# raviraina/grok

Measured on AMD Instinct MI355X. Metric: Mpixels/s encode+decode, 8K RGB 5/3 lossless + 9/7 lossy, 1/2/4/8 GPU, higher is better.
Workload: dtype int32 (5/3) + f32 (9/7)

## Files before the change

grok_amd/csrc/gk_engine.cpp:

```cpp
#include <hip/hip_runtime.h>

#include <algorithm>
#include <array>
#include <tuple>
#include <cmath>
#include <cstdarg>
#include <cstdlib>
#include <cstdio>
#include <cstring>
#include <memory>
#include <string>
#include <atomic>
#include <chrono>
#include <condition_variable>
#include <functional>
#include <mutex>
#include <thread>
#include <unordered_map>
#include <vector>
#include <queue>
#include <map>
#include <climits>
#include <linux/futex.h>
#include <sys/syscall.h>
// ... 2833 lines not shown
            } else if (p > q) {
                const uint32_t new_max = h.sgnd ? 1u << (p - 1) : (1u << p) - 1;
                const uint32_t old_max = h.sgnd ? 1u << (q - 1) : (1u << q) - 1;
                h.op = GK_PIX_SCALE;
                h.scale = (float)new_max / (float)old_max;
            } else if (p < q) {
                h.op = GK_PIX_SHIFT;
                h.shift = q - p;
            }
        }
    }
    return D;
}

}

struct DevBuf {
    void* p = nullptr; size_t cap = 0;
    void* get(size_t n) {
        if (n > cap) {
            if (p) (void)hipFree(p);
            p = nullptr; cap = 0;
            size_t c = std::max(n, (size_t)1 << 20);
            HIPCHK(hipMalloc(&p, c));
            cap = c;
        }
        return p;
    }
    ~DevBuf() { if (p) (void)hipFree(p); }
};
struct HostBuf {
    void* p = nullptr; size_t cap = 0;
    void* get(size_t n) {
        if (n > cap) {
            if (p) (void)hipHostFree(p);
            p = nullptr; cap = 0;
            size_t c = std::max(n, (size_t)1 << 20);
            HIPCHK(hipHostMalloc(&p, c, 0));
            cap = c;
        }
        return p;
    }
    ~HostBuf() { if (p) (void)hipHostFree(p); }
};

struct gk_ctx {
    uint32_t dec_layers = 0;
    bool dec_colour = true, col_inner = false, col_whole = false;
    uint32_t dec_display = 0;
    bool disp_inner = false;
    std::vector<gk_precision> dec_prec;
    bool out_inner = false;
    struct PixDst { void* pixels; size_t row_bytes; };
    const PixDst* pix = nullptr;
    DisplayOut hdr_disp;
    Jp2Colour hdr_col;
    ColourOut hdr_out;
    uint32_t hdr_ncs = 0;
    std::vector<uint8_t> col_blob;
    bool dwt_partial = false;
    uint32_t dec_reduce = 0;
    bool win_whole_tile = false;
    int device = 0;
    bool registered = false;
    hipStream_t st = nullptr;
    hipStream_t aux[3] = {nullptr, nullptr, nullptr};
    hipEvent_t xev[6];
    std::string err;
    gk_timings tm{};
    std::string plan_key;
    Plan plan;
    DevBuf arena;
    DevBuf bytes;
    DevBuf dblocks;
    DevBuf dpasses;
    DevBuf dinfo;
    DevBuf dseg;
    DevBuf dout;
    DevBuf dplanes;
    DevBuf derr;
    DevBuf dsym, dsymoff, dpassend, dcminfo;
    DevBuf dmsstate, dseglen;
    DevBuf dscratch, dnmse, dord, dweight, dord_enc;
    HostBuf hinfo, hseg, hhdr, hpasses, hord, hweight, hord_enc;
    DevBuf dstage1, dstage2;
    DevBuf dcol_src, dcol_out, dcol_tab;
    DevBuf dpix_src, dpix_out;
    DevBuf dicc_tab;
    std::vector<uint8_t> icc_blob;
    DevBuf dpix_in;
    HostBuf hstage1, hstage2;
    int16_t* nmse_tab = nullptr;
    hipEvent_t ev[32];
    bool blocks_uploaded = false;
    uint32_t enc_b0 = 0, enc_b1 = 0;
    std::vector<uint8_t> enc_dx, enc_dy;
    EncColour enc_col;
    std::vector<uint8_t> enc_jp2h;
    std::vector<uint32_t> hdr_dx, hdr_dy, hdr_prec, hdr_sgnd;
    bool enc_rc = false;
    std::vector<std::pair<uint32_t, uint32_t>> native_qcd, band_qcd;
    std::vector<gk_band_result> rb_bands;
    std::vector<gk_block_result> rb_blocks;
    std::vector<gk_pass_result> rb_passes;
    std::vector<uint8_t> rb_data;
};

static void set_params(Params& P, const gk_cparameters* cp, uint32_t nc) {
    for (int i = 0; i < GK_MAXRLVLS; ++i) { P.prcw[i] = 15; P.prch[i] = 15; }
    if (!cp) return;
    if (cp->numresolution > GK_MAXRLVLS) throw GkError("numresolution must be at most 33");
    if (cp->res_spec > GK_MAXRLVLS) throw GkError("res_spec must be at most 33");
    P.numres = cp->numresolution ? cp->numresolution : 6;
    P.cbw = (uint32_t)floorlog2(cp->cblockw_init ? cp->cblockw_init : 64);
    P.cbh = (uint32_t)floorlog2(cp->cblockh_init ? cp->cblockh_init : 64);
    P.irrev = cp->irreversible ? 1 : 0;
    P.mct = cp->mct;
    P.numgbits = cp->numgbits ? cp->numgbits : 2;
    P.nlayers = cp->numlayers ? cp->numlayers : 1;
    if (P.nlayers > GK_MAX_LAYERS) P.nlayers = GK_MAX_LAYERS;
    P.quality = cp->allocationByQuality != 0;
    for (uint32_t l = 0; l < GK_MAX_LAYERS; ++l) {
        P.rates[l] = (l < P.nlayers && !P.quality && cp->layer_rate[l] > 0.0) ? cp->layer_rate[l] : 0.0;
        P.dist[l] = (l < P.nlayers && P.quality && cp->layer_distortion[l] > 0.0) ? cp->layer_distortion[l] : 0.0;
    }
    if (cp->csty & ~7u) throw GkError("unknown coding style bits (csty)");
    P.sop_eph = cp->csty & 6u;
    P.write_com = cp->write_comment;
    P.comments.clear();
    if (cp->num_comments > GK_NUM_COMMENTS) throw GkError("at most 256 comments");
    uint32_t kept = 0;
    for (uint32_t i = 0; i < cp->num_comments; ++i)
        if (cp->comment_len[i] && cp->comment[i]) ++kept;
    for (uint32_t i = 0; i < kept; ++i) {
        if (!cp->comment_len[i] || !cp->comment[i]) continue;
        if (cp->comment_len[i] > 65531) throw GkError("comment longer than a COM marker holds (65531 bytes)");
        P.comments.push_back({cp->is_binary_comment[i] ? 0u : 1u, std::string(cp->comment[i], cp->comment_len[i])});
    }
    P.cblk_sty = cp->cblk_sty;
    if (cp->prog_order < 0 || cp->prog_order > 4) throw GkError("unknown progression order");
    P.prog = (uint32_t)cp->prog_order;
    P.roishift.clear();
    if (cp->roi_compno >= 0 && (uint32_t)cp->roi_compno < nc && cp->roi_shift) {
        if (cp->roi_shift >= 32) throw GkError("ROI shift must be below 32");
        P.roishift.assign(nc, 0);
        P.roishift[(size_t)cp->roi_compno] = (uint8_t)cp->roi_shift;
    }
    if (cp->numpocs > 32) throw GkError("at most 32 progression order changes");
    P.pocs.clear();
    for (uint32_t i = 0; i < cp->numpocs; ++i) {
        const gk_poc& g = cp->pocs[i];
        if (g.prog < 0 || g.prog > 4 || g.resE > GK_MAXRLVLS || g.resS >= g.resE || g.compS >= g.compE || !g.layE ||
            g.layE > 65535 || g.compE > 16384)
            throw GkError("bad progression order change");
        Poc e; e.rs = g.resS; e.cs = g.compS; e.lye = g.layE; e.re = g.resE; e.ce = g.compE; e.prog = (uint32_t)g.prog;
        P.pocs.push_back(e);
    }
    P.tp_div = cp->enableTilePartGeneration ? cp->newTilePartProgressionDivider : 0;
    if (P.tp_div && P.tp_div != 'L' && P.tp_div != 'R' && P.tp_div != 'C')
        throw GkError("tile-part divider must be L, R or C");
    if (cp->tile_size_on) {
        if (!cp->t_width || !cp->t_height) throw GkError("tile size must be non-zero when tiling is on");
        P.tw = cp->t_width; P.th = cp->t_height;
    }
    P.tlm = cp->writeTLM != 0; P.plt = cp->writePLT != 0;
    if (cp->cod_format != 0 && cp->cod_format != 2) throw GkError("cod_format must be GRK_CODEC_J2K (0) or GRK_CODEC_JP2 (2)");
    P.jp2 = cp->cod_format == 2;
// ... 342 lines not shown
        for (uint32_t c = 0; c < P.nc; ++c) {
            const Region& R = RGg[P.group_of[c]];
            const uint8_t* first = (const uint8_t*)comps[c] + (size_t)R.y0 * strides[c] * es;
            if (comps_on_device) { src[c] = first; sstr[c] = strides[c]; continue; }
            HIPCHK(hipMemcpy2DAsync(dp + o * es, (size_t)R.w * es, first, (size_t)strides[c] * es, (size_t)R.w * es, R.h,
                                    hipMemcpyHostToDevice, st));
            src[c] = dp + o * es; sstr[c] = R.w;
            o += (size_t)R.w * R.h;
        }
    }
    launch_check(__LINE__);
    HIPCHK(hipEventRecord(ctx->ev[1], st));
    int32_t shift = P.sgnd ? 0 : (1 << (P.prec - 1));
    auto planeA = [&](uint32_t c) { return arena + (size_t)c * 2 * RG.plane; };
    auto planeAf = [&](uint32_t c) { return reinterpret_cast<float*>(planeA(c)); };
    const bool mct3 = P.mct3();
    if (mct3 && (sstr[1] != sstr[0] || sstr[2] != sstr[0])) throw GkError("the first three components must share a stride");
    L1Io io;
    const bool fused = P.p.numres > 1 && P.l1_fusable;
    if (fused) {
        io.stype = stype; io.mct3 = mct3; io.shift.assign(P.nc, shift);
        io.planes.assign(src.begin(), src.end());
        io.strides = sstr;
    } else {
        auto cw = [&](uint32_t c) { return RGg[P.group_of[c]].w; };
        auto ch = [&](uint32_t c) { return RGg[P.group_of[c]].h; };
        if (!P.p.irrev) {
            if (mct3) gk_launch_dc_rct_fwd(st, stype, src[0], src[1], src[2], sstr[0], planeA(0), planeA(1), planeA(2), RG.stride, cw(0), ch(0), shift);
            for (uint32_t c = mct3 ? 3 : 0; c < P.nc; ++c) gk_launch_dc_fwd(st, stype, src[c], sstr[c], planeA(c), RG.stride, cw(c), ch(c), shift);
        } else {
            if (mct3) gk_launch_dc_ict_fwd(st, stype, src[0], src[1], src[2], sstr[0], planeAf(0), planeAf(1), planeAf(2), RG.stride, cw(0), ch(0), shift);
            for (uint32_t c = mct3 ? 3 : 0; c < P.nc; ++c) gk_launch_dc_fwd_f(st, stype, src[c], sstr[c], planeAf(c), RG.stride, cw(c), ch(c), shift);
        }
    }
    launch_check(__LINE__);
    HIPCHK(hipEventRecord(ctx->ev[2], st));
    run_dwt(ctx, RG, true, jb, je, 0, 0xffffffffu, fused ? &io : nullptr);
    if (const char* dp = getenv("GK_DUMP_DWT")) {
        std::vector<int32_t> hv((size_t)P.nc * 2 * RG.plane);
        HIPCHK(hipMemcpyAsync(hv.data(), arena, hv.size() * 4, hipMemcpyDeviceToHost, st));
        HIPCHK(hipStreamSynchronize(st));
        if (FILE* f = fopen(dp, "wb")) {
            const uint32_t hd[4] = {P.nc, RG.stride, RG.h, RG.w};
            fwrite(hd, 4, 4, f);
            fwrite(hv.data(), 4, hv.size(), f);
            fclose(f);
        }
    }
    launch_check(__LINE__);
    HIPCHK(hipEventRecord(ctx->ev[3], st));
    const bool do_rc = P.p.rate_control();
    const uint64_t slot0 = P.blocks[b0].data_off;
    const uint64_t slot1 = b1 < nb ? P.blocks[b1].data_off : P.slot_bytes;
    const uint64_t slot_span = slot1 - slot0;
    uint8_t* dbytes = (uint8_t*)ctx->bytes.get(slot_span + (64u << 20));
    const uint32_t nbx = std::max(nbr, 1u);
    GkBlock* dblk = (GkBlock*)ctx->dblocks.get(sizeof(GkBlock) * nbx);
    GkPass* dps = (GkPass*)ctx->dpasses.get(sizeof(GkPass) * GK_MAX_PASSES * (size_t)nbx);
    uint32_t* dinfo = (uint32_t*)ctx->dinfo.get(16 * (size_t)nbx + 16);
    int* derr = (int*)ctx->derr.get(64);
    uint32_t* dpcount = (uint32_t*)(derr + 4);
    uint8_t* dsym = P.p.ht() ? nullptr : (uint8_t*)ctx->dsym.get(P.sym_off[b1] - P.sym_off[b0] + 256);
    uint64_t* dsymoff = (uint64_t*)ctx->dsymoff.get(8 * ((size_t)nbr + 1));
    uint32_t* dpe = (uint32_t*)ctx->dpassend.get(4 * GK_MAX_PASSES * (size_t)nbx);
    uint32_t* dcm = (uint32_t*)ctx->dcminfo.get(8 * (size_t)nbx);
    int32_t* dnmse = do_rc ? (int32_t*)ctx->dnmse.get(4 * GK_MAX_PASSES * (size_t)nbx) : nullptr;
    if (!ctx->blocks_uploaded || ctx->enc_b0 != b0 || ctx->enc_b1 != b1 || ctx->enc_rc != do_rc) {
        GkBlock* hb = (GkBlock*)ctx->hpasses.get(sizeof(GkBlock) * nbx + 8 * ((size_t)nbr + 1));
        uint64_t* hso = (uint64_t*)(hb + nbx);
        for (uint32_t i = 0; i < nbr; ++i) {
            hb[i] = P.blocks[b0 + i];
            hb[i].band_off = relocate(P, group_region(P, RG, P.groups[P.group_of[hb[i].comp]]), hb[i].band_off);
            hb[i].stride = RG.stride;
            hb[i].data_off -= slot0;
            hb[i].flags = (uint8_t)((hb[i].flags & ~2u) | (do_rc ? 2u : 0u));
        }
        for (uint32_t i = 0; i <= nbr; ++i) hso[i] = P.sym_off[b0 + i] - P.sym_off[b0];
        HIPCHK(hipMemcpyAsync(dblk, hb, sizeof(GkBlock) * nbr, hipMemcpyHostToDevice, st));
        HIPCHK(hipMemcpyAsync(dsymoff, hso, 8 * ((size_t)nbr + 1), hipMemcpyHostToDevice, st));
        HIPCHK(hipStreamSynchronize(st));
        ctx->blocks_uploaded = true; ctx->enc_b0 = b0; ctx->enc_b1 = b1; ctx->enc_rc = do_rc;
    }
    HIPCHK(hipMemsetAsync(derr, 0, 64, st));
    const uint32_t nsolo_env = []() { const char* v = getenv("GK_T1ENC_SOLO"); return v ? (uint32_t)atoi(v) : 0u; }();
    if (P.p.ht()) {
        uint8_t* mel = (uint8_t*)ctx->dsym.get((size_t)nbx * GK_HT_MEL_CAP + 256);
        launch_check(__LINE__);
        HIPCHK(hipEventRecord(ctx->ev[8], st));
        gk_launch_ht_enc(st, arena, dblk, dbytes, mel, GK_HT_MEL_CAP, dinfo, nbr, derr, P.p.wide());
    } else if (P.p.t1_generic()) {
        uint8_t* mst = (uint8_t*)ctx->dmsstate.get(gk_t1ms_state_bytes(nbx));
        launch_check(__LINE__);
        HIPCHK(hipEventRecord(ctx->ev[8], st));
        gk_launch_t1_enc_ms(st, arena, dblk, dbytes, dps, dinfo, nbr, derr, ctx->nmse_tab, dpcount, mst, P.p.cblk_sty & 0x3f);
    } else if (nbr < 8192 || getenv("GK_T1ENC_SERIAL")) {
        gk_launch_t1_cm(st, arena, dblk, dsymoff, dsym, dpe, dcm, nbr, derr, ctx->nmse_tab, dnmse);
        launch_check(__LINE__);
        HIPCHK(hipEventRecord(ctx->ev[8], st));
        gk_launch_t1_mq(st, dsym, dsymoff, dpe, dcm, dblk, dbytes, dps, dinfo, nbr, derr, dnmse, dpcount, nullptr, 0,
                        0xffffffffu, std::min(nsolo_env, nbr));
    } else {
        uint32_t* dw = (uint32_t*)ctx->dweight.get(4 * (size_t)nbr);
        gk_launch_t1_weight(st, arena, dblk, dw, nbr);
        uint32_t* hw = (uint32_t*)ctx->hweight.get(4 * (size_t)nbr);
        HIPCHK(hipMemcpyAsync(hw, dw, 4 * (size_t)nbr, hipMemcpyDeviceToHost, st));
        HIPCHK(hipStreamSynchronize(st));
        uint32_t wmax = 1;
        for (uint32_t i = 0; i < nbr; ++i) wmax = std::max(wmax, hw[i]);
        const uint32_t kB = 4096;
        auto key = [&](uint32_t i) { return kB - 1 - (uint32_t)(((uint64_t)hw[i] * (kB - 1)) / wmax); };
        std::vector<uint32_t> start(kB + 1, 0);
        for (uint32_t i = 0; i < nbr; ++i) start[key(i)]++;
        for (uint32_t k = 0, acc = 0; k <= kB; ++k) { const uint32_t c = start[k]; start[k] = acc; acc += c; }
        uint32_t* ho = (uint32_t*)ctx->hord_enc.get(4 * (size_t)nbr);
        for (uint32_t i = 0; i < nbr; ++i) ho[start[key(i)]++] = i;
        uint32_t* dord = (uint32_t*)ctx->dord_enc.get(4 * (size_t)nbr);
        HIPCHK(hipMemcpyAsync(dord, ho, 4 * (size_t)nbr, hipMemcpyHostToDevice, st));
        static std::vector<double> frs[2];
        std::vector<double>& fr = frs[do_rc ? 1 : 0];
        if (fr.empty()) {
            const char* cv = getenv("GK_T1ENC_CUTS");
            std::string cs = cv ? cv : (do_rc ? "0.08,0.25" : "0.125,0.375");
            for (size_t q = 0; q < cs.size();) {
                size_t e = cs.find(',', q);
                if (e == std::string::npos) e = cs.size();
                const double f = atof(cs.substr(q, e - q).c_str());
                if (f > 0 && f < 1 && fr.size() < 3) fr.push_back(f);
                q = e + 1;
            }
        }
        std::vector<uint32_t> cut(1, 0);
        for (double f : fr) {
            const uint32_t c = (uint32_t)(nbr * f) / 256 * 256;
            if (c > cut.back() && c < nbr) cut.push_back(c);
        }
        cut.push_back(nbr);
        const int nch = (int)cut.size() - 1;
        for (int k = 0; k < nch; ++k) {
            const uint32_t base = cut[k], cnt = cut[k + 1] - cut[k];
            gk_launch_t1_cm(st, arena, dblk, dsymoff, dsym, dpe, dcm, nbr, derr, ctx->nmse_tab, dnmse, dord, base, cnt);
            if (k + 1 < nch) {
                HIPCHK(hipEventRecord(ctx->xev[k], st));
                HIPCHK(hipStreamWaitEvent(ctx->aux[k], ctx->xev[k], 0));
                gk_launch_t1_mq(ctx->aux[k], dsym, dsymoff, dpe, dcm, dblk, dbytes, dps, dinfo, nbr, derr, dnmse, dpcount,
                                dord, base, cnt, k == 0 ? std::min(nsolo_env, cnt) : 0u);
                HIPCHK(hipEventRecord(ctx->xev[3 + k], ctx->aux[k]));
            } else {
                launch_check(__LINE__);
                HIPCHK(hipEventRecord(ctx->ev[8], st));
                gk_launch_t1_mq(st, dsym, dsymoff, dpe, dcm, dblk, dbytes, dps, dinfo, nbr, derr, dnmse, dpcount, dord,
                                base, cnt);
            }
        }
        for (int k = 0; k + 1 < nch; ++k) HIPCHK(hipStreamWaitEvent(st, ctx->xev[3 + k], 0));
    }
    launch_check(__LINE__);
    HIPCHK(hipEventRecord(ctx->ev[4], st));
    static const bool eprof = getenv("GK_PROFILE") != nullptr;
    using eclk = std::chrono::steady_clock;
    auto ems = [](eclk::time_point a, eclk::time_point b) { return std::chrono::duration<double, std::milli>(b - a).count(); };
    const auto te0 = eclk::now();
    uint32_t* hinfo = (uint32_t*)ctx->hinfo.get(16 * (size_t)nb + 64);
    HIPCHK(hipMemcpyAsync(hinfo + 4 * (size_t)b0, dinfo, 16 * (size_t)nbr, hipMemcpyDeviceToHost, st));
    HIPCHK(hipMemcpyAsync(hinfo + 4 * (size_t)nb, derr, 32, hipMemcpyDeviceToHost, st));
    HIPCHK(hipStreamSynchronize(st));
    const uint32_t t1err = hinfo[4 * (size_t)nb], npass_total = hinfo[4 * (size_t)nb + 4];
    if (t1err) throw GkError(t1err & 2 ? "T1 symbol buffer overflow" : "T1 code-block slot overflow");
    const bool ht = P.p.ht();
    const GkPass* hpasses = nullptr;
    if ((do_rc || (P.p.cblk_sty & (GK_STY_LAZY | GK_STY_TERMALL))) && !ht) {
        GkPass* hp = (GkPass*)ctx->hpasses.get(sizeof(GkPass) * (size_t)std::max(npass_total, 1u));
        HIPCHK(hipMemcpyAsync(hp, dps, sizeof(GkPass) * (size_t)npass_total, hipMemcpyDeviceToHost, st));
        HIPCHK(hipStreamSynchronize(st));
        hpasses = hp;
    }
    if (blocks_only) {
        dump_blocks(ctx, hinfo, dps, npass_total, dbytes, slot0);
        *rc = 0;
        return 0;
    }

    std::vector<uint8_t> H;
    H.reserve(1 << 12);
    size_t tlm_pos = 0;
    write_main_header(H, P, &tlm_pos);
    const size_t rc_header_size = H.size() + (P.p.jp2 ? jp2_prefix_size(P, ctx->enc_jp2h) : 0);
    if (!with_header) H.clear();
    const auto te1 = eclk::now();
    if (const char* ds = getenv("GK_DUMP_SYMS"); ds && dsym && !P.p.t1_generic()) {
        std::vector<uint32_t> pe((size_t)GK_MAX_PASSES * nbr), cm(2 * (size_t)nbr), out(2 * (size_t)nbr);
        HIPCHK(hipMemcpy(pe.data(), dpe, 4 * pe.size(), hipMemcpyDeviceToHost));
        HIPCHK(hipMemcpy(cm.data(), dcm, 4 * cm.size(), hipMemcpyDeviceToHost));
        for (uint32_t i = 0; i < nbr; ++i) {
            out[2 * i] = cm[2 * i + 1] ? pe[(size_t)GK_MAX_PASSES * i + cm[2 * i + 1] - 1] : 0;
            out[2 * i + 1] = cm[2 * i];
        }
        if (FILE* f = fopen(ds, "wb")) { fwrite(out.data(), 4, out.size(), f); fclose(f); }
    }
    if (const char* dp = getenv("GK_DUMP_PASSES")) {
        if (FILE* f = fopen(dp, "wb")) {
            const uint32_t hdr[2] = {nb, npass_total};
            fwrite(hdr, 4, 2, f);
            fwrite(hinfo, 16, nb, f);
            if (hpasses) fwrite(hpasses, sizeof(GkPass), npass_total, f);
            fclose(f);
        }
    }
    T2Enc T2(P, hinfo, hpasses, tb, te);
    std::vector<T2Enc::Swallow> tsw(te - tb);
    if (te - tb == 1 || !P.p.rate_control()) {
        T2.allocate(rc_header_size);
        tsw[0] = T2.final_sw;
    } else {
        const bool par = te - tb >= host_pool().size();
        auto one = [&](size_t q) {
            const uint32_t t = tb + (uint32_t)q;
            T2Enc Tt(P, hinfo, hpasses, t, t + 1);
            Tt.serial = par;
            Tt.allocate(rc_header_size);
            tsw[q] = Tt.final_sw;
            const TileG& TG = P.tiles[t];
            std::copy(Tt.lnp.begin() + (size_t)TG.b0 * T2.L, Tt.lnp.begin() + (size_t)TG.b1 * T2.L,
                      T2.lnp.begin() + (size_t)TG.b0 * T2.L);
        };
        if (par) host_pool().run(te - tb, one);
        else for (uint32_t q = 0; q < te - tb; ++q) one(q);
    }
    const auto te2 = eclk::now();
// ... 2777 lines not shown
```

grok_amd/csrc/gk_launch.h:

```cpp
#pragma once
#include <hip/hip_runtime.h>
#include <stdint.h>
#include "gk_common.h"

#define GK_SAMPLE_DISPATCH(t, T, ...)                            \
    switch (t) {                                                 \
        case GK_U8: { typedef uint8_t T; __VA_ARGS__; break; }   \
        case GK_S8: { typedef int8_t T; __VA_ARGS__; break; }    \
        case GK_U16: { typedef uint16_t T; __VA_ARGS__; break; } \
        case GK_S16: { typedef int16_t T; __VA_ARGS__; break; }  \
        default: { typedef int32_t T; __VA_ARGS__; break; }      \
    }

void gk_launch_dc_rct_fwd(hipStream_t st, int stype, const void* r, const void* g, const void* b, uint32_t sin,
                          int32_t* y, int32_t* u, int32_t* v, uint32_t sout, uint32_t w, uint32_t h, int32_t shift);
void gk_launch_dc_fwd(hipStream_t st, int stype, const void* in, uint32_t sin, int32_t* out, uint32_t sout, uint32_t w,
                      uint32_t h, int32_t shift);
void gk_launch_rct_inv_dc(hipStream_t st, const int32_t* y, const int32_t* u, const int32_t* v, uint32_t sin, int stype,
                          void* r, void* g, void* b, uint32_t sout, uint32_t w, uint32_t h, int32_t shift,
                          int32_t mn, int32_t mx);
void gk_launch_dc_inv(hipStream_t st, const int32_t* in, uint32_t sin, int stype, void* out, uint32_t sout, uint32_t w,
                      uint32_t h, int32_t shift, int32_t mn, int32_t mx);
uint32_t gk_dwt_cpw(uint32_t wgs, uint32_t n, bool multi);
void gk_launch_dwt53_fwd(hipStream_t st, const int32_t* src, uint32_t sstride, int32_t* dst, uint32_t dstride,
                         uint32_t w, uint32_t h, GkTiles tb = GkTiles(), GkComps cs = GkComps());
void gk_launch_dwt53_inv(hipStream_t st, const int32_t* src, uint32_t sstride, int32_t* dst, uint32_t dstride,
                         uint32_t w, uint32_t h, GkTiles tb = GkTiles(), GkComps cs = GkComps());
void gk_launch_dwt53_fwd_l1(hipStream_t st, int stype, int nc, GkPtr3 in, uint32_t sin, int32_t* dst, uint64_t cstride,
                            uint32_t dstride, uint32_t w, uint32_t h, GkTiles tb, int32_t shift);
void gk_launch_dwt53_inv_l1(hipStream_t st, int stype, int nc, const int32_t* src, uint64_t cstride, uint32_t sstride,
                            GkPtr3 out, uint32_t ostride, GkWin win, uint32_t w, uint32_t h, GkTiles tb, int32_t shift,
                            int32_t mn, int32_t mx);
void gk_launch_gather(hipStream_t st, const uint8_t* src, uint8_t* dst, const uint64_t* seg, uint32_t nseg);
void gk_launch_t1_cm(hipStream_t st, const int32_t* coef, const GkBlock* blocks, const uint64_t* sym_off, uint8_t* sym,
                     uint32_t* pass_end, uint32_t* cm_info, uint32_t nblocks, int* err, const int16_t* nmse_tab,
                     int32_t* pass_nmse, const uint32_t* order = nullptr, uint32_t base = 0, uint32_t count = 0xffffffffu);
void gk_launch_t1_mq(hipStream_t st, const uint8_t* sym, const uint64_t* sym_off, const uint32_t* pass_end,
                     const uint32_t* cm_info, const GkBlock* blocks, uint8_t* bytes, GkPass* passes, uint32_t* info,
                     uint32_t nblocks, int* err, const int32_t* pass_nmse, uint32_t* pass_counter,
                     const uint32_t* order = nullptr, uint32_t base = 0, uint32_t count = 0xffffffffu,
                     uint32_t nsolo = 0);
void gk_launch_t1_weight(hipStream_t st, const int32_t* coef, const GkBlock* blocks, uint32_t* weight, uint32_t nblocks);
uint32_t gk_t1dec_lanes();
void gk_t1dec_stats(uint64_t out[5]);
struct GkSoloPlan { uint32_t waves; int forced; float ratio; };
GkSoloPlan gk_t1dec_solo_plan(uint32_t nblocks, uint32_t lanes);
void gk_launch_t1_dec(hipStream_t st, const uint8_t* bytes, const GkBlock* blocks, const uint32_t* order,
                      uint64_t* scratch, const uint64_t* wave_off, uint32_t nblocks, uint32_t nsolo);
void gk_launch_t1_recon(hipStream_t st, const GkBlock* blocks, const uint32_t* ids, const uint32_t* pos,
                        const uint64_t* scratch, const uint64_t* wave_off, int32_t* coef, uint32_t nblocks,
                        uint32_t maxnp);
void gk_launch_dwt_any(hipStream_t st, bool irrev, bool forward, int32_t* in, int32_t* out, uint32_t stride, uint32_t w,
                       uint32_t h, uint32_t px, uint32_t py, GkTiles tb, GkComps cs, bool partial = false);
void gk_launch_t1_enc_ms(hipStream_t st, const int32_t* coef, const GkBlock* blocks, uint8_t* bytes, GkPass* passes,
                         uint32_t* info, uint32_t nblocks, int* err, const int16_t* nmse_tab, uint32_t* pass_counter,
                         uint8_t* state, uint32_t sty);
void gk_launch_t1_dec_ms(hipStream_t st, const uint8_t* bytes, const GkBlock* blocks, const uint32_t* seglen, int32_t* coef,
                         uint32_t nblocks, uint8_t* state, uint32_t sty);
size_t gk_t1ms_state_bytes(uint32_t nblocks);
void gk_launch_dc_ict_fwd(hipStream_t st, int stype, const void* r, const void* g, const void* b, uint32_t sin, float* y,
                          float* u, float* v, uint32_t sout, uint32_t w, uint32_t h, int32_t shift);
void gk_launch_dc_fwd_f(hipStream_t st, int stype, const void* in, uint32_t sin, float* out, uint32_t sout, uint32_t w,
                        uint32_t h, int32_t shift);
void gk_launch_ict_inv_dc(hipStream_t st, const float* y, const float* u, const float* v, uint32_t sin, int stype, void* r,
                          void* g, void* b, uint32_t sout, uint32_t w, uint32_t h, int32_t shift, int32_t mn,
                          int32_t mx);
void gk_launch_dc_inv_f(hipStream_t st, const float* in, uint32_t sin, int stype, void* out, uint32_t sout, uint32_t w,
                        uint32_t h, int32_t shift, int32_t mn, int32_t mx);
void gk_launch_dwt97_fwd(hipStream_t st, const float* src, uint32_t sstride, float* dst, uint32_t dstride, uint32_t w,
                         uint32_t h, GkTiles tb = GkTiles(), GkComps cs = GkComps());
void gk_launch_dwt97_inv(hipStream_t st, const float* src, uint32_t sstride, float* dst, uint32_t dstride, uint32_t w,
                         uint32_t h, GkTiles tb = GkTiles(), GkComps cs = GkComps());
void gk_launch_dwt97_fwd_l1(hipStream_t st, int stype, int nc, GkPtr3 in, uint32_t sin, float* dst, uint64_t cstride,
                            uint32_t dstride, uint32_t w, uint32_t h, GkTiles tb, int32_t shift);
void gk_launch_dwt97_inv_l1(hipStream_t st, int stype, int nc, const float* src, uint64_t cstride, uint32_t sstride,
                            GkPtr3 out, uint32_t ostride, GkWin win, uint32_t w, uint32_t h, GkTiles tb, int32_t shift,
                            int32_t mn, int32_t mx);
void gk_launch_ht_enc(hipStream_t st, const int32_t* coef, const GkBlock* blocks, uint8_t* bytes, uint8_t* mel_scratch,
                      uint32_t mel_cap, uint32_t* info, uint32_t nblocks, int* err, bool wide = false);
void gk_launch_ht_dec(hipStream_t st, const uint8_t* bytes, const GkBlock* blocks, const uint32_t* ids, int32_t* coef,
                      uint32_t nblocks, int* err, bool wide = false);
struct GkPalChan {
    void* dst;
    const void* src;
    uint32_t dst_stride, src_stride;
    uint32_t col, direct;
};
struct GkPalArgs {
    const void* idx;
    uint32_t idx_stride;
    uint32_t w, h;
    const GkPalChan* chans;
    uint32_t nchan, npal;
    const uint32_t* table;
    uint32_t ne, entry_words, elem_bytes;
    uint32_t vec_store;
    uint32_t rows;
};
#define GK_PAL_PIX 8
#define GK_PAL_LDS_BYTES 65536u
uint32_t gk_pal_entry_words(uint32_t npc, uint32_t elem_bytes);
int gk_launch_jp2_palette(hipStream_t st, int stype, int dtype, const GkPalArgs& args);
enum GkYccMode { GK_YCC_444 = 0, GK_YCC_422 = 1, GK_YCC_420 = 2, GK_YCC_ESYCC = 3 };
struct GkYccArgs {
    const void* y; const void* cb; const void* cr;
    uint32_t ys, cs;
    void* dst[3];
    uint32_t ds[3];
    uint32_t w, h;
    uint32_t mode;
    uint32_t ofx, ofy;
    int32_t offset, upb;
    uint32_t flip_cb, flip_cr;
    uint32_t vec_store;
    uint32_t rows;
};
void gk_launch_ycc_rgb(hipStream_t st, int stype, int dtype, const GkYccArgs& args);
struct GkCmykArgs {
    const void* src[4];
    uint32_t ss;
    void* dst[3];
    uint32_t ds[3];
    uint32_t w, h;
    float scale[4];
    uint32_t vec_store;
// ... 80 lines not shown
```

grok_amd/csrc/gk_t1enc.hip:

```cpp
#include <hip/hip_runtime.h>
#include <stdint.h>
#include "gk_common.h"
#include "gk_t1_common.h"
#include <algorithm>
#include <type_traits>
#include <cstdlib>

#define SYM_PER_PLANE 11264u

__device__ __forceinline__ uint32_t win6(uint64_t col, uint32_t s) {
    return (uint32_t)((s ? (col >> (4 * s - 1)) : (col << 1)) & 63u);
}

__device__ __forceinline__ uint32_t lane_prev(uint32_t v) {
    return (uint32_t)__builtin_amdgcn_update_dpp(0, (int)v, 0x138, 0xf, 0xf, false);
}
__device__ __forceinline__ uint32_t lane_next(uint32_t v) {
    return (uint32_t)__builtin_amdgcn_update_dpp(0, (int)v, 0x130, 0xf, 0xf, false);
}
__device__ __forceinline__ uint32_t wave_excl_scan(uint32_t v, uint32_t& total) {
    int inc = (int)v;
    inc += __builtin_amdgcn_update_dpp(0, inc, 0x111, 0xf, 0xf, false);
    inc += __builtin_amdgcn_update_dpp(0, inc, 0x112, 0xf, 0xf, false);
    inc += __builtin_amdgcn_update_dpp(0, inc, 0x114, 0xf, 0xf, false);
    inc += __builtin_amdgcn_update_dpp(0, inc, 0x118, 0xf, 0xf, false);
    inc += __builtin_amdgcn_update_dpp(0, inc, 0x142, 0xa, 0xf, false);
    inc += __builtin_amdgcn_update_dpp(0, inc, 0x143, 0xc, 0xf, false);
    total = (uint32_t)__builtin_amdgcn_readlane(inc, 63);
    return (uint32_t)inc - v;
}

__device__ __forceinline__ uint32_t nb9(uint32_t L, uint32_t C, uint32_t R, int r) {
    return ((L >> r) & 7u) | (((C >> r) & 7u) << 3) | (((R >> r) & 7u) << 6);
}
__device__ __forceinline__ uint32_t sc8(uint32_t fs, uint32_t fn) { return (fs & 0xaau) | ((fn >> 1) & 0x55u); }
__host__ __device__ constexpr uint32_t zc_of_nb9(uint32_t i) {
    return (i & 1u) | (((i >> 3) & 1u) << 1) | (((i >> 6) & 1u) << 2) | (((i >> 1) & 1u) << 3) | (((i >> 4) & 1u) << 4) |
           (((i >> 7) & 1u) << 5) | (((i >> 2) & 1u) << 6) | (((i >> 5) & 1u) << 7) | (((i >> 8) & 1u) << 8);
}
__host__ __device__ constexpr uint32_t sc_of_sc8(uint32_t i) {
    return (i & 3u) | (((i >> 6) & 3u) << 2) | (((i >> 2) & 3u) << 4) | (((i >> 4) & 3u) << 6);
}
struct alignas(16) CmTabs {
    uint8_t zc[4][512];
    uint8_t sc[256];
};
constexpr CmTabs make_cm_tabs() {
    CmTabs t{};
    for (uint32_t o = 0; o < 4; ++o)
        for (uint32_t i = 0; i < 512; ++i) t.zc[o][i] = zc_rule(o, zc_of_nb9(i));
    for (uint32_t i = 0; i < 256; ++i) t.sc[i] = sc_rule(sc_of_sc8(i));
    return t;
}
__constant__ CmTabs c_cm_tabs = make_cm_tabs();

struct alignas(16) CmLds {
    uint8_t zc[512];
    uint8_t sc[256];
};
struct CmRcLds {
    int16_t nm[4][128];
};

__device__ __forceinline__ int32_t wave_sum(int32_t v) {
#pragma unroll
    for (int o = 32; o > 0; o >>= 1) v += __shfl_xor(v, o);
    return v;
}

template <bool RC>
__global__ __launch_bounds__(64) void k_t1_cm(const int32_t* __restrict__ coef, const GkBlock* __restrict__ blocks,
                                              const uint64_t* __restrict__ sym_off, uint8_t* __restrict__ sym,
                                              uint32_t* __restrict__ pass_end, uint32_t* __restrict__ cm_info,
                                              uint32_t nblocks, int* err, const int16_t* __restrict__ nmse_tab,
                                              int32_t* __restrict__ pass_nmse, const uint32_t* __restrict__ order,
                                              uint32_t base, uint32_t count) {
    __shared__ CmLds L;
    __shared__ typename std::conditional<RC, CmRcLds, char>::type R;
    if (blockIdx.x >= count) return;
    const uint32_t b = order ? order[base + blockIdx.x] : base + blockIdx.x;
    if (b >= nblocks) return;
    const int lane = threadIdx.x;
    const GkBlock B = blocks[b];
    const uint32_t w = B.w, h = B.h;
    reinterpret_cast<uint2*>(L.zc)[lane] = reinterpret_cast<const uint2*>(c_cm_tabs.zc[B.orient & 3])[lane];
    reinterpret_cast<uint32_t*>(L.sc)[lane] = reinterpret_cast<const uint32_t*>(c_cm_tabs.sc)[lane];
    const bool irrev = B.flags & 1;
    uint32_t m[64];
    uint64_t negcol = 0;
    uint32_t mx = 0;
#pragma unroll
    for (int y = 0; y < 64; ++y) {
        int32_t raw = 0;
        uint32_t a = 0;
        if (y < (int)h && lane < (int)w) {
            raw = coef[B.band_off + (size_t)y * B.stride + lane];
            if (irrev) a = (uint32_t)fabsf(rintf((__int_as_float(raw) / B.step) * 64.0f));
            else a = (uint32_t)(raw < 0 ? -raw : raw) * 64u;
        }
        m[y] = a;
        mx = a > mx ? a : mx;
        negcol |= (uint64_t)(raw < 0) << y;
    }
    if (const uint32_t rs = B.flags >> 3) {
        mx = 0;
#pragma unroll
        for (int y = 0; y < 64; ++y) {
            m[y] = ((m[y] >> 6) << (6 + rs)) | (m[y] & 63u);
            mx = m[y] > mx ? m[y] : mx;
        }
    }
    if constexpr (RC) {
        for (int i = lane; i < 512; i += 64) R.nm[i >> 7][i & 127] = nmse_tab[i];
    }
#pragma unroll
    for (int o = 32; o > 0; o >>= 1) { uint32_t t = __shfl_xor(mx, o); mx = t > mx ? t : mx; }
    uint32_t numbps = 0;
    if (mx) { uint32_t t = 32 - __clz(mx); numbps = t <= 6 ? 0 : t - 6; }
    __syncthreads();
    if (numbps == 0) {
        if (lane == 0) { cm_info[2 * b] = 0; cm_info[2 * b + 1] = 0; }
        return;
    }
    const uint64_t base_off = sym_off[b];
    const uint64_t cap = sym_off[b + 1] - base_off;
    if ((uint64_t)numbps * SYM_PER_PLANE > cap) {
        if (lane == 0) { atomicOr(err, 2); cm_info[2 * b] = 0; cm_info[2 * b + 1] = 0; }
        return;
    }
    uint8_t* S = sym + base_off;
    uint32_t* PE = pass_end + (size_t)b * GK_MAX_PASSES;
    const uint64_t validcol = (lane < (int)w) ? ((h >= 64) ? ~0ull : ((1ull << h) - 1)) : 0ull;
    const uint32_t nstripes = (h + 3) >> 2;
    uint64_t sig = 0, mu = 0;
    uint32_t pos = 0, passno = 0;
    int32_t acc = 0;
    auto nm_rows = [&](uint64_t mask, int t, int bp) __attribute__((always_inline)) {
        if constexpr (RC) {
            const int16_t* tab = R.nm[bp > 0 ? t : t + 1];
#pragma unroll
            for (int g = 0; g < 8; ++g) {
                const uint32_t gm = (uint32_t)(mask >> (8 * g)) & 0xffu;
                if (__any(gm != 0)) {
#pragma unroll
                    for (int k = 0; k < 8; ++k)
                        if ((gm >> k) & 1) acc += tab[(m[8 * g + k] >> bp) & 127];
                }
            }
        }
    };
    auto end_pass = [&]() {
        if (lane == 0) PE[passno] = pos;
        if constexpr (RC) {
            int32_t t = wave_sum(acc);
            if (lane == 0) pass_nmse[(size_t)b * GK_MAX_PASSES + passno] = t;
            acc = 0;
        }
        ++passno;
    };

    for (int bpno = (int)numbps - 1; bpno >= 0; --bpno) {
        uint64_t bitcol = 0;
#pragma unroll
        for (int y = 0; y < 64; ++y) bitcol |= (uint64_t)((m[y] >> (bpno + 6)) & 1u) << y;
        uint64_t vis = 0;
        const uint64_t sigPrev = sig;
        if (bpno != (int)numbps - 1) {
            for (uint32_t s = 0; s < nstripes; ++s) {
                const uint32_t sh = 4 * s;
                const uint32_t Wc = win6(sig, s), Nc = win6(negcol, s);
                uint32_t pk = Wc | (Nc << 6);
                const uint32_t pL = lane_prev(pk), pR = lane_next(pk);
                const uint32_t WL = pL & 63, NL = (pL >> 6) & 63, WR = pR & 63, NR = (pR >> 6) & 63;
                const uint32_t valid4 = (uint32_t)(validcol >> sh) & 15u;
                const uint32_t cand = ~(Wc >> 1) & valid4;
                const uint32_t bit4 = (uint32_t)(bitcol >> sh) & 15u;
                const uint32_t A = ((WL | (WL >> 1) | (WL >> 2)) | (WR | (WR >> 1) | (WR >> 2)) | Wc | (Wc >> 2)) & 15u;
                auto F = [&](uint32_t in, uint32_t& cd) -> uint32_t {
                    uint32_t x = A | ((in | (in << 1) | (in >> 1)) & 15u);
                    uint32_t c0 = cand & x & 1u, n0 = c0 & bit4;
                    uint32_t c1 = cand & (x | (n0 << 1)) & 2u, n1 = c1 & bit4;
                    uint32_t c2 = cand & (x | (n1 << 1)) & 4u, n2 = c2 & bit4;
                    uint32_t c3 = cand & (x | (n2 << 1)) & 8u, n3 = c3 & bit4;
                    cd = c0 | c1 | c2 | c3;
                    return n0 | n1 | n2 | n3;
                };
                uint32_t cd, in = 0;
                uint32_t ns = F(0, cd);
                while (true) {
                    in = lane_prev(ns);
                    uint32_t cd2, ns2 = F(in, cd2);
                    bool ch = ns2 != ns;
                    ns = ns2; cd = cd2;
                    if (!__any(ch)) break;
                }
                const uint32_t Lt = WL | (in << 1), Cn = ns << 1;
                uint32_t cnt = __popc(cd) + __popc(ns);
                uint32_t total, off = wave_excl_scan(cnt, total);
                uint8_t* o = S + pos + off;
#pragma unroll
                for (int r = 0; r < 4; ++r) {
                    if ((cd >> r) & 1) {
                        const uint32_t d = (bit4 >> r) & 1;
                        const uint32_t fs = nb9(Lt, Wc | (Cn & ((2u << r) - 1)), WR, r);
                        *o++ = (uint8_t)(((CTX_ZC + L.zc[fs]) << 1) | d);
                        if (d) {
                            const uint32_t e = L.sc[sc8(fs, nb9(NL, Nc, NR, r))];
                            const uint32_t sg = (Nc >> (r + 1)) & 1;
                            *o++ = (uint8_t)(((CTX_SC + (e & 15)) << 1) | (sg ^ (e >> 4)));
                        }
                    }
                }
                pos += total;
                sig |= (uint64_t)ns << sh;
                vis |= (uint64_t)cd << sh;
            }
            nm_rows(sig & ~sigPrev, 0, bpno);
            end_pass();
            for (uint32_t s = 0; s < nstripes; ++s) {
                const uint32_t sh = 4 * s;
                const uint32_t Wc = win6(sig, s);
                const uint32_t pL = lane_prev(Wc), pR = lane_next(Wc);
                const uint32_t nb = ((pL | (pL >> 1) | (pL >> 2)) | (pR | (pR >> 1) | (pR >> 2)) | Wc | (Wc >> 2)) & 15u;
                const uint32_t mr = (uint32_t)(sigPrev >> sh) & 15u;
                const uint32_t mu4 = (uint32_t)(mu >> sh) & 15u;
                const uint32_t bit4 = (uint32_t)(bitcol >> sh) & 15u;
                uint32_t total, off = wave_excl_scan(__popc(mr), total);
                uint8_t* o = S + pos + off;
#pragma unroll
                for (int r = 0; r < 4; ++r) {
                    if ((mr >> r) & 1) {
                        uint32_t cx = ((mu4 >> r) & 1) ? CTX_MAG + 2 : (((nb >> r) & 1) ? CTX_MAG + 1 : CTX_MAG);
                        *o++ = (uint8_t)((cx << 1) | ((bit4 >> r) & 1));
                    }
                }
                pos += total;
            }
            nm_rows(sigPrev, 2, bpno);
            mu |= sigPrev;
            end_pass();
        }
        const uint64_t sigCu = sig;
        for (uint32_t s = 0; s < nstripes; ++s) {
            const uint32_t sh = 4 * s;
            const uint32_t Wc = win6(sig, s), Nc = win6(negcol, s);
            const uint32_t valid4 = (uint32_t)(validcol >> sh) & 15u;
            const uint32_t vis4 = (uint32_t)(vis >> sh) & 15u;
            const uint32_t bit4 = (uint32_t)(bitcol >> sh) & 15u;
            const uint32_t cl = ~(Wc >> 1) & ~vis4 & valid4;
            const uint32_t nc = cl & bit4;
            uint32_t pk = Wc | (Nc << 6) | (nc << 12);
            const uint32_t pL = lane_prev(pk), pR = lane_next(pk);
            const uint32_t WL = pL & 63, NL = (pL >> 6) & 63, ncL = (pL >> 12) & 15;
            const uint32_t WR = pR & 63, NR = (pR >> 6) & 63;
            const uint32_t Lt = WL | (ncL << 1), Cn = nc << 1;
            const bool agg = (valid4 == 15u) && (cl == 15u) && ((Lt | WR | (Wc & 0x21u)) == 0);
            uint32_t rl = nc ? (uint32_t)__ffs(nc) - 1 : 4u;
            uint32_t cnt;
            uint32_t codemask;
            if (agg) {
                if (rl == 4) { cnt = 1; codemask = 0; }
                else {
                    codemask = cl & ~((2u << rl) - 1);
                    cnt = 3 + 1 + __popc(codemask) + __popc(nc & codemask);
                }
            } else {
                codemask = cl;
                cnt = __popc(cl) + __popc(nc);
            }
            uint32_t total, off = wave_excl_scan(cnt, total);
            uint8_t* o = S + pos + off;
            if (agg) {
                *o++ = (uint8_t)((CTX_AGG << 1) | (rl != 4 ? 1 : 0));
                if (rl != 4) {
                    *o++ = (uint8_t)((CTX_UNI << 1) | (rl >> 1));
                    *o++ = (uint8_t)((CTX_UNI << 1) | (rl & 1));
                    const uint32_t sg = (Nc >> (rl + 1)) & 1;
                    *o++ = (uint8_t)((CTX_SC << 1) | sg);
                }
            }
#pragma unroll
            for (int r = 0; r < 4; ++r) {
                if ((codemask >> r) & 1) {
                    const uint32_t d = (bit4 >> r) & 1;
                    const uint32_t fs = nb9(Lt, Wc | (Cn & ((2u << r) - 1)), WR, r);
                    *o++ = (uint8_t)(((CTX_ZC + L.zc[fs]) << 1) | d);
                    if (d) {
                        const uint32_t e = L.sc[sc8(fs, nb9(NL, Nc, NR, r))];
                        const uint32_t sg = (Nc >> (r + 1)) & 1;
                        *o++ = (uint8_t)(((CTX_SC + (e & 15)) << 1) | (sg ^ (e >> 4)));
                    }
                }
            }
            pos += total;
            sig |= (uint64_t)nc << sh;
        }
        nm_rows(sig & ~sigCu, 0, bpno);
        end_pass();
    }
    if (lane == 0) { cm_info[2 * b] = numbps; cm_info[2 * b + 1] = passno; }
}

#define MQ_RING_DW 32
struct MqLane {
    uint32_t a, c, ct;
    int32_t bp;
    uint32_t cur;
    uint8_t* out;
    uint32_t cap;
    uint32_t lf;
    uint32_t pcx1, pne1, epref;
};
struct MqLds {
    uint32_t tab[96];
    uint32_t ctx[20][64];
    uint32_t ring[64][MQ_RING_DW + 1];
};

__device__ __forceinline__ void mq_line_store(MqLane& q, MqLds& L, int lane, uint32_t li) {
    const uint32_t o = (li & 1) * 16;
    uint8_t* dst = q.out + (size_t)li * 64;
    if ((li + 1) * 64 <= q.cap) {
#pragma unroll
        for (int i = 0; i < 4; ++i)
            *(uint4*)(dst + 16 * i) = make_uint4(L.ring[lane][o + 4 * i], L.ring[lane][o + 4 * i + 1],
                                                 L.ring[lane][o + 4 * i + 2], L.ring[lane][o + 4 * i + 3]);
    } else {
        for (uint32_t i = 0; i < 16 && li * 64 + 4 * i + 4 <= q.cap; ++i) *(uint32_t*)(dst + 4 * i) = L.ring[lane][o + i];
    }
}
__device__ __forceinline__ void mq_lines_out(MqLane& q, MqLds& L, int lane) {
    const uint32_t cl = (uint32_t)max(q.bp, 0) >> 6;
// ... 323 lines not shown
        cur4 = nxt4; nxt4 = pre;
        mq_lines_out(q, L, lane);
    }
    if (npasses && q.bp >= 0 && (uint32_t)q.bp < q.cap) {
        const uint32_t bp = (uint32_t)q.bp, cl = bp >> 6;
        reinterpret_cast<uint8_t*>(&L.ring[lane][0])[bp & (4 * MQ_RING_DW - 1)] = (uint8_t)q.cur;
        if (cl > q.lf) mq_line_store(q, L, lane, q.lf);
        const uint32_t o = (cl & 1) * 16, k = (bp >> 2) & 15;
        for (uint32_t i = 0; i <= k; ++i) *(uint32_t*)(q.out + (size_t)cl * 64 + 4 * i) = L.ring[lane][o + i];
    }
    if (!has) return;
    if (npasses == 0) { info[4 * b] = 0; info[4 * b + 1] = 0; info[4 * b + 2] = 0; info[4 * b + 3] = 0; return; }
    __threadfence();
    const uint32_t nbytes = (uint32_t)q.bp;
    uint32_t last = nbytes;
    for (int k = (int)npasses; k > 0;) {
        GkPass& ps = P[--k];
        if (ps.rate > last) ps.rate = last; else last = ps.rate;
    }
    uint32_t prev = 0;
    for (uint32_t k = 0; k < npasses; ++k) {
        GkPass& ps = P[k];
        if (ps.rate > 0 && ps.rate <= q.cap && q.out[ps.rate - 1] == 0xff) ps.rate--;
        ps.len = ps.rate - prev;
        prev = ps.rate;
    }
    info[4 * b] = numbps;
    info[4 * b + 1] = npasses;
    info[4 * b + 2] = P[npasses - 1].rate;
    info[4 * b + 3] = poff;
    if (q.bp > 0 && (uint32_t)q.bp > q.cap) atomicOr(err, 1);
#undef pe_lds_at
}

#include "gk_launch.h"
void gk_launch_t1_cm(hipStream_t st, const int32_t* coef, const GkBlock* blocks, const uint64_t* sym_off, uint8_t* sym,
                     uint32_t* pass_end, uint32_t* cm_info, uint32_t nblocks, int* err, const int16_t* nmse_tab,
                     int32_t* pass_nmse, const uint32_t* order, uint32_t base, uint32_t count) {
    if (!nblocks) return;
    if (count == 0xffffffffu) count = nblocks;
    if (!count) return;
    if (pass_nmse)
        hipLaunchKernelGGL(k_t1_cm<true>, dim3(count), dim3(64), 0, st, coef, blocks, sym_off, sym, pass_end, cm_info,
                           nblocks, err, nmse_tab, pass_nmse, order, base, count);
    else
        hipLaunchKernelGGL(k_t1_cm<false>, dim3(count), dim3(64), 0, st, coef, blocks, sym_off, sym, pass_end,
                           cm_info, nblocks, err, nmse_tab, pass_nmse, order, base, count);
}

__global__ __launch_bounds__(64) void k_t1_weight(const int32_t* __restrict__ coef, const GkBlock* __restrict__ blocks,
                                                  uint32_t* __restrict__ weight, uint32_t nblocks) {
    const uint32_t b = blockIdx.x;
    if (b >= nblocks) return;
    const int lane = threadIdx.x;
    const GkBlock B = blocks[b];
    const bool irrev = B.flags & 1;
    uint32_t mx = 0, nbits = 0;
    if (lane < (int)B.w)
#pragma unroll 4
        for (uint32_t y = 0; y < B.h; y += 4) {
            const int32_t raw = coef[B.band_off + (size_t)y * B.stride + lane];
            const uint32_t a0 = irrev ? (uint32_t)fabsf(rintf((__int_as_float(raw) / B.step) * 64.0f))
                                      : (uint32_t)(raw < 0 ? -raw : raw) * 64u;
            const uint32_t a = ((a0 >> 6) << (6 + (B.flags >> 3))) | (a0 & 63u);
            mx = a > mx ? a : mx;
            nbits += (a >> 6) ? 32u - __clz(a >> 6) : 0u;
        }
#pragma unroll
    for (int o = 32; o > 0; o >>= 1) {
        const uint32_t t = __shfl_xor(mx, o); mx = t > mx ? t : mx;
        nbits += __shfl_xor(nbits, o);
    }
    if (lane == 0) {
        const uint32_t t = mx ? 32 - __clz(mx) : 0;
        const uint32_t planes = t <= 6 ? 0 : t - 6;
        const uint32_t rows = (B.h + 3) / 4;
        weight[b] = planes * B.w * B.h * 5u + (uint32_t)((3ull * nbits * B.h) / (rows ? rows : 1));
    }
}
void gk_launch_t1_weight(hipStream_t st, const int32_t* coef, const GkBlock* blocks, uint32_t* weight, uint32_t nblocks) {
    if (!nblocks) return;
    hipLaunchKernelGGL(k_t1_weight, dim3(nblocks), dim3(64), 0, st, coef, blocks, weight, nblocks);
}
void gk_launch_t1_mq(hipStream_t st, const uint8_t* sym, const uint64_t* sym_off, const uint32_t* pass_end,
                     const uint32_t* cm_info, const GkBlock* blocks, uint8_t* bytes, GkPass* passes, uint32_t* info,
                     uint32_t nblocks, int* err, const int32_t* pass_nmse, uint32_t* pass_counter, const uint32_t* order,
                     uint32_t base, uint32_t count, uint32_t nsolo) {
    if (!nblocks) return;
    if (count == 0xffffffffu) count = nblocks;
    if (!count) return;
    nsolo = std::min((nsolo + 3) / 4 * 4, (count + 3) / 4 * 4);
    static const uint32_t nl = [] {
        const char* v = getenv("GK_T1ENC_LANES");
        const int n = v ? atoi(v) : 64;
        return (uint32_t)(n < 1 ? 1 : (n > 64 ? 64 : n));
    }();
    const size_t pe = (size_t)(GK_MAX_PASSES + 1) * nl * 4 * 4;
    const size_t lds = std::max(pe, (size_t)163840 - 4 * sizeof(MqLds));
    const uint32_t rest = count > nsolo ? count - nsolo : 0;
    hipLaunchKernelGGL(k_t1_mq, dim3(nsolo / 4 + (rest + 4 * nl - 1) / (4 * nl)), dim3(256), lds, st, sym, sym_off,
                       pass_end, cm_info, blocks, bytes, passes, info, nblocks, err, pass_nmse, pass_counter, nl, order,
                       base, count, nsolo);
}
```

Measured before the change: 1800.

## Sort T1 encode blocks by weight on GPU and skip empty stripes in cm kernel

Replaces the host round trip (device-to-host weight copy, stream sync, CPU bucket sort, upload) with a single-workgroup GPU counting-sort kernel, so the encoder no longer stalls the stream. Bucketing now uses a fixed shift of the weight instead of normalising by the maximum, which can make the ordering coarser or uneven. The context-modelling kernel gets wave-uniform early-outs for stripes with no candidates, a simpler propagation fixpoint loop, a readfirstlane on numbps, and a waves-per-EU attribute. A default of 64 solo blocks is enabled for rate-controlled encodes. The atomic-based scatter makes the order within a bucket nondeterministic.

```diff
diff --git a/grok_amd/csrc/gk_engine.cpp b/grok_amd/csrc/gk_engine.cpp
--- a/grok_amd/csrc/gk_engine.cpp
+++ b/grok_amd/csrc/gk_engine.cpp
@@ -2939,7 +2939,7 @@
     DevBuf dsym, dsymoff, dpassend, dcminfo;
     DevBuf dmsstate, dseglen;
     DevBuf dscratch, dnmse, dord, dweight, dord_enc;
-    HostBuf hinfo, hseg, hhdr, hpasses, hord, hweight, hord_enc;
+    HostBuf hinfo, hseg, hhdr, hpasses, hord;
     DevBuf dstage1, dstage2;
     DevBuf dcol_src, dcol_out, dcol_tab;
     DevBuf dpix_src, dpix_out;
@@ -3448,7 +3448,8 @@
         ctx->blocks_uploaded = true; ctx->enc_b0 = b0; ctx->enc_b1 = b1; ctx->enc_rc = do_rc;
     }
     HIPCHK(hipMemsetAsync(derr, 0, 64, st));
-    const uint32_t nsolo_env = []() { const char* v = getenv("GK_T1ENC_SOLO"); return v ? (uint32_t)atoi(v) : 0u; }();
+    const char* nsolo_str = getenv("GK_T1ENC_SOLO");
+    const uint32_t nsolo_env = nsolo_str ? (uint32_t)atoi(nsolo_str) : 0u;
     if (P.p.ht()) {
         uint8_t* mel = (uint8_t*)ctx->dsym.get((size_t)nbx * GK_HT_MEL_CAP + 256);
         launch_check(__LINE__);
@@ -3468,20 +3469,8 @@
     } else {
         uint32_t* dw = (uint32_t*)ctx->dweight.get(4 * (size_t)nbr);
         gk_launch_t1_weight(st, arena, dblk, dw, nbr);
-        uint32_t* hw = (uint32_t*)ctx->hweight.get(4 * (size_t)nbr);
-        HIPCHK(hipMemcpyAsync(hw, dw, 4 * (size_t)nbr, hipMemcpyDeviceToHost, st));
-        HIPCHK(hipStreamSynchronize(st));
-        uint32_t wmax = 1;
-        for (uint32_t i = 0; i < nbr; ++i) wmax = std::max(wmax, hw[i]);
-        const uint32_t kB = 4096;
-        auto key = [&](uint32_t i) { return kB - 1 - (uint32_t)(((uint64_t)hw[i] * (kB - 1)) / wmax); };
-        std::vector<uint32_t> start(kB + 1, 0);
-        for (uint32_t i = 0; i < nbr; ++i) start[key(i)]++;
-        for (uint32_t k = 0, acc = 0; k <= kB; ++k) { const uint32_t c = start[k]; start[k] = acc; acc += c; }
-        uint32_t* ho = (uint32_t*)ctx->hord_enc.get(4 * (size_t)nbr);
-        for (uint32_t i = 0; i < nbr; ++i) ho[start[key(i)]++] = i;
         uint32_t* dord = (uint32_t*)ctx->dord_enc.get(4 * (size_t)nbr);
-        HIPCHK(hipMemcpyAsync(dord, ho, 4 * (size_t)nbr, hipMemcpyHostToDevice, st));
+        gk_launch_t1_order(st, dw, dord, nbr);
         static std::vector<double> frs[2];
         std::vector<double>& fr = frs[do_rc ? 1 : 0];
         if (fr.empty()) {
@@ -3502,6 +3491,7 @@
         }
         cut.push_back(nbr);
         const int nch = (int)cut.size() - 1;
+        const uint32_t nsolo = nsolo_str ? nsolo_env : (do_rc ? 64u : 0u);
         for (int k = 0; k < nch; ++k) {
             const uint32_t base = cut[k], cnt = cut[k + 1] - cut[k];
             gk_launch_t1_cm(st, arena, dblk, dsymoff, dsym, dpe, dcm, nbr, derr, ctx->nmse_tab, dnmse, dord, base, cnt);
@@ -3509,7 +3499,7 @@
                 HIPCHK(hipEventRecord(ctx->xev[k], st));
                 HIPCHK(hipStreamWaitEvent(ctx->aux[k], ctx->xev[k], 0));
                 gk_launch_t1_mq(ctx->aux[k], dsym, dsymoff, dpe, dcm, dblk, dbytes, dps, dinfo, nbr, derr, dnmse, dpcount,
-                                dord, base, cnt, k == 0 ? std::min(nsolo_env, cnt) : 0u);
+                                dord, base, cnt, k == 0 ? std::min(nsolo, cnt) : 0u);
                 HIPCHK(hipEventRecord(ctx->xev[3 + k], ctx->aux[k]));
             } else {
                 launch_check(__LINE__);
diff --git a/grok_amd/csrc/gk_launch.h b/grok_amd/csrc/gk_launch.h
--- a/grok_amd/csrc/gk_launch.h
+++ b/grok_amd/csrc/gk_launch.h
@@ -41,6 +41,7 @@
                      const uint32_t* order = nullptr, uint32_t base = 0, uint32_t count = 0xffffffffu,
                      uint32_t nsolo = 0);
 void gk_launch_t1_weight(hipStream_t st, const int32_t* coef, const GkBlock* blocks, uint32_t* weight, uint32_t nblocks);
+void gk_launch_t1_order(hipStream_t st, const uint32_t* weight, uint32_t* order, uint32_t nblocks);
 uint32_t gk_t1dec_lanes();
 void gk_t1dec_stats(uint64_t out[5]);
 struct GkSoloPlan { uint32_t waves; int forced; float ratio; };
diff --git a/grok_amd/csrc/gk_t1enc.hip b/grok_amd/csrc/gk_t1enc.hip
--- a/grok_amd/csrc/gk_t1enc.hip
+++ b/grok_amd/csrc/gk_t1enc.hip
@@ -69,7 +69,7 @@
 }
 
 template <bool RC>
-__global__ __launch_bounds__(64) void k_t1_cm(const int32_t* __restrict__ coef, const GkBlock* __restrict__ blocks,
+__global__ __launch_bounds__(64) __attribute__((amdgpu_waves_per_eu(4, 4))) void k_t1_cm(const int32_t* __restrict__ coef, const GkBlock* __restrict__ blocks,
                                               const uint64_t* __restrict__ sym_off, uint8_t* __restrict__ sym,
                                               uint32_t* __restrict__ pass_end, uint32_t* __restrict__ cm_info,
                                               uint32_t nblocks, int* err, const int16_t* __restrict__ nmse_tab,
@@ -117,6 +117,7 @@
     for (int o = 32; o > 0; o >>= 1) { uint32_t t = __shfl_xor(mx, o); mx = t > mx ? t : mx; }
     uint32_t numbps = 0;
     if (mx) { uint32_t t = 32 - __clz(mx); numbps = t <= 6 ? 0 : t - 6; }
+    numbps = (uint32_t)__builtin_amdgcn_readfirstlane((int)numbps);
     __syncthreads();
     if (numbps == 0) {
         if (lane == 0) { cm_info[2 * b] = 0; cm_info[2 * b + 1] = 0; }
@@ -169,11 +170,12 @@
             for (uint32_t s = 0; s < nstripes; ++s) {
                 const uint32_t sh = 4 * s;
                 const uint32_t Wc = win6(sig, s), Nc = win6(negcol, s);
+                const uint32_t valid4 = (uint32_t)(validcol >> sh) & 15u;
+                const uint32_t cand = ~(Wc >> 1) & valid4;
+                if (!__any(Wc != 0) || !__any(cand != 0)) continue;
                 uint32_t pk = Wc | (Nc << 6);
                 const uint32_t pL = lane_prev(pk), pR = lane_next(pk);
                 const uint32_t WL = pL & 63, NL = (pL >> 6) & 63, WR = pR & 63, NR = (pR >> 6) & 63;
-                const uint32_t valid4 = (uint32_t)(validcol >> sh) & 15u;
-                const uint32_t cand = ~(Wc >> 1) & valid4;
                 const uint32_t bit4 = (uint32_t)(bitcol >> sh) & 15u;
                 const uint32_t A = ((WL | (WL >> 1) | (WL >> 2)) | (WR | (WR >> 1) | (WR >> 2)) | Wc | (Wc >> 2)) & 15u;
                 auto F = [&](uint32_t in, uint32_t& cd) -> uint32_t {
@@ -188,11 +190,10 @@
                 uint32_t cd, in = 0;
                 uint32_t ns = F(0, cd);
                 while (true) {
-                    in = lane_prev(ns);
-                    uint32_t cd2, ns2 = F(in, cd2);
-                    bool ch = ns2 != ns;
-                    ns = ns2; cd = cd2;
-                    if (!__any(ch)) break;
+                    const uint32_t in2 = lane_prev(ns);
+                    if (!__any(in2 != in)) break;
+                    in = in2;
+                    ns = F(in, cd);
                 }
                 const uint32_t Lt = WL | (in << 1), Cn = ns << 1;
                 uint32_t cnt = __popc(cd) + __popc(ns);
@@ -219,10 +220,11 @@
             end_pass();
             for (uint32_t s = 0; s < nstripes; ++s) {
                 const uint32_t sh = 4 * s;
+                const uint32_t mr = (uint32_t)(sigPrev >> sh) & 15u;
+                if (!__any(mr != 0)) continue;
                 const uint32_t Wc = win6(sig, s);
                 const uint32_t pL = lane_prev(Wc), pR = lane_next(Wc);
                 const uint32_t nb = ((pL | (pL >> 1) | (pL >> 2)) | (pR | (pR >> 1) | (pR >> 2)) | Wc | (Wc >> 2)) & 15u;
-                const uint32_t mr = (uint32_t)(sigPrev >> sh) & 15u;
                 const uint32_t mu4 = (uint32_t)(mu >> sh) & 15u;
                 const uint32_t bit4 = (uint32_t)(bitcol >> sh) & 15u;
                 uint32_t total, off = wave_excl_scan(__popc(mr), total);
@@ -248,6 +250,7 @@
             const uint32_t vis4 = (uint32_t)(vis >> sh) & 15u;
             const uint32_t bit4 = (uint32_t)(bitcol >> sh) & 15u;
             const uint32_t cl = ~(Wc >> 1) & ~vis4 & valid4;
+            if (!__any(cl != 0)) continue;
             const uint32_t nc = cl & bit4;
             uint32_t pk = Wc | (Nc << 6) | (nc << 12);
             const uint32_t pL = lane_prev(pk), pR = lane_next(pk);
@@ -737,6 +740,37 @@
     if (!nblocks) return;
     hipLaunchKernelGGL(k_t1_weight, dim3(nblocks), dim3(64), 0, st, coef, blocks, weight, nblocks);
 }
+#define T1_ORD_KEYS 8192u
+__global__ __launch_bounds__(1024) void k_t1_order(const uint32_t* __restrict__ weight, uint32_t* __restrict__ order,
+                                                   uint32_t nblocks) {
+    __shared__ uint32_t cnt[T1_ORD_KEYS];
+    __shared__ uint32_t part[1024];
+    const uint32_t t = threadIdx.x;
+    constexpr uint32_t per = T1_ORD_KEYS / 1024;
+    auto bucket = [](uint32_t w) { return T1_ORD_KEYS - 1 - min(w >> 7, T1_ORD_KEYS - 1); };
+    for (uint32_t i = t; i < T1_ORD_KEYS; i += 1024) cnt[i] = 0;
+    __syncthreads();
+    for (uint32_t i = t; i < nblocks; i += 1024) atomicAdd(&cnt[bucket(weight[i])], 1u);
+    __syncthreads();
+    uint32_t s = 0;
+    for (uint32_t k = 0; k < per; ++k) s += cnt[per * t + k];
+    part[t] = s;
+    __syncthreads();
+    for (uint32_t o = 1; o < 1024; o <<= 1) {
+        const uint32_t v = t >= o ? part[t - o] : 0;
+        __syncthreads();
+        part[t] += v;
+        __syncthreads();
+    }
+    uint32_t run = part[t] - s;
+    for (uint32_t k = 0; k < per; ++k) { const uint32_t c = cnt[per * t + k]; cnt[per * t + k] = run; run += c; }
+    __syncthreads();
+    for (uint32_t i = t; i < nblocks; i += 1024) order[atomicAdd(&cnt[bucket(weight[i])], 1u)] = i;
+}
+void gk_launch_t1_order(hipStream_t st, const uint32_t* weight, uint32_t* order, uint32_t nblocks) {
+    if (!nblocks) return;
+    hipLaunchKernelGGL(k_t1_order, dim3(1), dim3(1024), 0, st, weight, order, nblocks);
+}
 void gk_launch_t1_mq(hipStream_t st, const uint8_t* sym, const uint64_t* sym_off, const uint32_t* pass_end,
                      const uint32_t* cm_info, const GkBlock* blocks, uint8_t* bytes, GkPass* passes, uint32_t* info,
                      uint32_t nblocks, int* err, const int32_t* pass_nmse, uint32_t* pass_counter, const uint32_t* order,
```

Result: no change. 1786 (-0.8%).
